# mapbox/robosat

Hardware: AMD Instinct MI355X
Metric: 512x512 tiles/sec train+predict, 1/2/4/8 MI355X; mIoU vs CPU ref (higher is better)
Workload: dtype f32; 1 GPU; rs predict ResNet50-UNet, bs=16 3x512x512 fp32 per GPU, 2 classes (BASELINE configs[1]); parallelism=tiles sharded over 1 rank(s), no collective

## Files before the change

### robosat_amd/csrc/common.h

```cpp
#pragma once
#include <hip/hip_runtime.h>
#include <stdint.h>

#include "../../include/robosat_hip.h"

typedef float f32x4 __attribute__((ext_vector_type(4)));
typedef float f32x16 __attribute__((ext_vector_type(16)));
typedef __bf16 bf16_t;
typedef __bf16 bf16x4 __attribute__((ext_vector_type(4)));
typedef __bf16 bf16x8 __attribute__((ext_vector_type(8)));
typedef unsigned int u32x2 __attribute__((ext_vector_type(2)));
typedef unsigned int u32x4 __attribute__((ext_vector_type(4)));
typedef short s16x4 __attribute__((ext_vector_type(4)));
typedef short s16x8 __attribute__((ext_vector_type(8)));

__device__ __forceinline__ f32x4 rs_ld4(const float* p) { return *reinterpret_cast<const f32x4*>(p); }
__device__ __forceinline__ f32x4 rs_ld4(const bf16_t* p) {
  return __builtin_convertvector(*reinterpret_cast<const bf16x4*>(p), f32x4);
}
__device__ __forceinline__ void rs_st4(float* p, f32x4 v) { *reinterpret_cast<f32x4*>(p) = v; }
__device__ __forceinline__ void rs_st4(bf16_t* p, f32x4 v) {
  *reinterpret_cast<bf16x4*>(p) = __builtin_convertvector(v, bf16x4);
}
__device__ __forceinline__ float rs_ld1(const float* p) { return *p; }
__device__ __forceinline__ float rs_ld1(const bf16_t* p) { return (float)*p; }

template <int V>
struct rs_vecf {
  float v[V];
};
template <int V, typename T>
__device__ __forceinline__ rs_vecf<V> rs_ldv(const T* p) {
  rs_vecf<V> r;
  if constexpr (V == 4) {
    const f32x4 t = rs_ld4(p);
#pragma unroll
    for (int e = 0; e < 4; ++e) r.v[e] = t[e];
  } else if constexpr (sizeof(T) == 2) {
    const bf16x8 t = *reinterpret_cast<const bf16x8*>(p);
#pragma unroll
    for (int e = 0; e < 8; ++e) r.v[e] = (float)t[e];
  } else {
    const f32x4 a = *reinterpret_cast<const f32x4*>(p), b = *(reinterpret_cast<const f32x4*>(p) + 1);
#pragma unroll
    for (int e = 0; e < 4; ++e) r.v[e] = a[e], r.v[4 + e] = b[e];
  }
  return r;
}
template <int V, typename T>
__device__ __forceinline__ void rs_stv(T* p, const rs_vecf<V>& r) {
  if constexpr (V == 4) {
    rs_st4(p, f32x4{r.v[0], r.v[1], r.v[2], r.v[3]});
  } else if constexpr (sizeof(T) == 2) {
    bf16x8 t;
#pragma unroll
    for (int e = 0; e < 8; ++e) t[e] = (bf16_t)r.v[e];
    *reinterpret_cast<bf16x8*>(p) = t;
  } else {
    *reinterpret_cast<f32x4*>(p) = f32x4{r.v[0], r.v[1], r.v[2], r.v[3]};
    *(reinterpret_cast<f32x4*>(p) + 1) = f32x4{r.v[4], r.v[5], r.v[6], r.v[7]};
  }
}

__device__ __forceinline__ void rs_ld_row32(const bf16_t* p, float (&v)[32]) {
  bf16x8 t[4];
#pragma unroll
  for (int j = 0; j < 4; ++j) t[j] = *reinterpret_cast<const bf16x8*>(p + j * 8);
#pragma unroll
  for (int j = 0; j < 4; ++j)
#pragma unroll
    for (int e = 0; e < 8; ++e) v[j * 8 + e] = (float)t[j][e];
}
__device__ __forceinline__ void rs_ld_row32(const float* p, float (&v)[32]) {
  f32x4 t[8];
#pragma unroll
  for (int j = 0; j < 8; ++j) t[j] = *reinterpret_cast<const f32x4*>(p + j * 4);
#pragma unroll
  for (int j = 0; j < 8; ++j)
#pragma unroll
    for (int e = 0; e < 4; ++e) v[j * 4 + e] = t[j][e];
}
__device__ __forceinline__ void rs_st_row32(bf16_t* p, const float (&v)[32]) {
#pragma unroll
  for (int j = 0; j < 4; ++j) {
    bf16x8 t;
#pragma unroll
    for (int e = 0; e < 8; ++e) t[e] = (bf16_t)v[j * 8 + e];
    *reinterpret_cast<bf16x8*>(p + j * 8) = t;
  }
}
__device__ __forceinline__ void rs_st_row32(float* p, const float (&v)[32]) {
#pragma unroll
  for (int j = 0; j < 8; ++j) {
    f32x4 t;
#pragma unroll
    for (int e = 0; e < 4; ++e) t[e] = v[j * 4 + e];
    *reinterpret_cast<f32x4*>(p + j * 4) = t;
  }
}

#define RS_LAUNCH_RESULT() ((int)hipGetLastError())

__device__ __forceinline__ void rs_lds_writes_done() { asm volatile("s_waitcnt lgkmcnt(0)" ::: "memory"); }

__device__ __forceinline__ int rs_xcd_remap(int b, int nwg) {
  const int xcd = b & 7, k = b >> 3;
  const int q = nwg >> 3, r = nwg & 7;
  const int base = (xcd < r) ? xcd * (q + 1) : r * (q + 1) + (xcd - r) * q;
  return base + k;
}

__device__ __forceinline__ float rs_xor16_sum(float v) {
  float a = v, b = v;
  asm("s_nop 1\n\tv_permlane16_swap_b32 %0, %1" : "+v"(a), "+v"(b));
  return a + b;
}
__device__ __forceinline__ float rs_xor32_sum(float v) {
  float a = v, b = v;
  asm("s_nop 1\n\tv_permlane32_swap_b32 %0, %1" : "+v"(a), "+v"(b));
  return a + b;
}

__device__ __forceinline__ float rs_row16_sum(float v) {
  v += __builtin_bit_cast(float, __builtin_amdgcn_update_dpp(0, __builtin_bit_cast(int, v), 0x128, 0xf, 0xf, false));
  v += __builtin_bit_cast(float, __builtin_amdgcn_update_dpp(0, __builtin_bit_cast(int, v), 0x124, 0xf, 0xf, false));
  v += __builtin_bit_cast(float, __builtin_amdgcn_update_dpp(0, __builtin_bit_cast(int, v), 0x122, 0xf, 0xf, false));
  v += __builtin_bit_cast(float, __builtin_amdgcn_update_dpp(0, __builtin_bit_cast(int, v), 0x121, 0xf, 0xf, false));
  return v;
}

__device__ __forceinline__ float rs_wave_sum(float v) {
#pragma unroll
  for (int o = 32; o > 0; o >>= 1) v += __shfl_xor(v, o, 64);
  return v;
}

__device__ __forceinline__ double rs_wave_sum(double v) {
#pragma unroll
  for (int o = 32; o > 0; o >>= 1) v += __shfl_xor(v, o, 64);
  return v;
}

static inline int rs_cdiv(long a, long b) { return (int)((a + b - 1) / b); }

inline int rs_cu_count() {
  static const int n = [] {
    int dev = 0, cus = 0;
    if (hipGetDevice(&dev) != hipSuccess || hipDeviceGetAttribute(&cus, hipDeviceAttributeMultiprocessorCount, dev) != hipSuccess || cus <= 0)
      cus = 256;
    return cus;
  }();
  return n;
}

struct rs_fastdiv {
  unsigned int mul;
  unsigned int shift;
  unsigned int div;
};

static inline rs_fastdiv rs_make_fastdiv(unsigned int d) {
  rs_fastdiv f;
  unsigned int s = 0;
  while ((1ull << s) < d) ++s;
  f.shift = s;
  f.mul = (unsigned int)((((1ull << s) - d) << 32) / d + 1);
  f.div = d;
  return f;
}

__host__ __device__ __forceinline__ unsigned int rs_div(unsigned int n, const rs_fastdiv f) {
#if defined(__HIP_DEVICE_COMPILE__)
  return (__umulhi(n, f.mul) + n) >> f.shift;
#else
  return (unsigned int)((((unsigned long long)n * f.mul) >> 32) + n) >> f.shift;
#endif
}

struct RsKnobs {
  int conv_tile = -1;
  int conv_rowb = 0;
  int conv_big = 1;
  int conv_min256 = 384;
  int conv_halo = 1;
  int conv_halo_min = 192;
  int conv_halo512 = -1;
  int conv_splitk = -1;
  int conv1x1_ew = -1;
  int conv1x1_np = 0;
  int conv1x1_ew_bf16 = 0;
  int halo_ko = 0;
  int wgrad_f32_phase = 1;
  int wgrad_f32_dma = -1;
  int wgrad_f32_blocks = 2048;
  int wgrad_f32_wino = 1;
  int wgrad_f32_wino_blocks = 1024;
  int wgrad_f32_wino33 = 1;
  int wgrad_f32_wino33_blocks = 256;
  int wgrad_blocks = 96;
  int wgrad_blocks_phase = 1536;
  int wgrad_phase4 = 1;
  int wgrad_blocks_phase4 = 256;
  int wgrad_ring = 3;
  int lovasz_xcd = 1;
  int wino_wide = 1;
  int wino_pixel = 1;
  int grow_fused = 0;
};
__attribute__((visibility("hidden"))) RsKnobs& rs_knobs();

__attribute__((visibility("hidden"))) int rs_wgrad_thin_plan(const rs_conv_desc* d, int* blocks, int* slices);
__attribute__((visibility("hidden"))) int rs_wgrad_thin_launch(const rs_conv_desc* d, const void* dy, const void* src,
                                                               float* partial, void* stream);

__attribute__((visibility("hidden"))) int rs_conv_thin_bf16_launch(int mode, const void* src, const void* wgt, const void* mask,
                                                                   void* out, int N, int Hs, int Ws, int relu, void* stream);

__attribute__((visibility("hidden"))) long rs_reduce_scratch_floats(long n, int splits);
__attribute__((visibility("hidden"))) int rs_reduce_splits(const float* ws, float* out, long n, int splits, float* scratch,
                                                           void* stream);

__attribute__((visibility("hidden"))) int rs_conv_dma_f32(const rs_conv_desc* d, const float* src1, const float* src2,
                                                          const float* weight, const float* scale, const float* shift,
                                                          const float* residual, const float* relu_mask, float* out,
                                                          void* stream);
__attribute__((visibility("hidden"))) int rs_conv_dma_tile(const rs_conv_desc* d);
```

### robosat_amd/csrc/conv_wino_f32.hip

```cpp
#define RS_CONV_INSTANTIATE
#include "conv_igemm_dma_kernel.h"

namespace {

struct WinoArgs {
  const float* src1;
  const float* src2;
  const float* u;
  float* out;
  int N, Hs, Ws, C1, C2, Cout;
  int TY, TX;
  int BBY, BBX;
  int nsub;
  int ncb;
  int relu;
  float* out2;
  const float* mask1;
  const float* mask2;
  int csplit;
};

template <int PB, bool PIX = false>
struct WinoGeom {
  static constexpr int HW = PIX ? 10 : 2 * PB + 1;
  static constexpr int PITCH = HW;
  static constexpr int HALF = PB + 1;
  static constexpr int SBROWS = (HW * PITCH + 7) / 8 * 8;
};

template <int PB>
__device__ __forceinline__ int wino_lane_tile(int l) {
  if constexpr (PB == 8) return ((l & 1) << 1) | (((l >> 1) & 1) << 2) | ((l >> 2) & 1) | (l & 8);
  return ((l & 1) << 1) | (((l >> 1) & 1) << 3) | ((l >> 2) & 1) | (((l >> 3) & 1) << 2);
}
__device__ __forceinline__ int wino_lane_pixel_y(int l) { return l & 3; }
__device__ __forceinline__ int wino_lane_pixel_x(int l) { return (l >> 2) & 3; }
typedef float f32x2 __attribute__((ext_vector_type(2)));
__device__ __forceinline__ f32x2 pk_sub(f32x2 a, f32x2 b) {
  f32x2 d;
  asm("v_pk_add_f32 %0, %1, %2 neg_lo:[0,1] neg_hi:[0,1]" : "=v"(d) : "v"(a), "v"(b));
  return d;
}
__device__ __forceinline__ int wino_lane_now() {
  int l;
  asm volatile("v_mbcnt_lo_u32_b32 %0, -1, 0\n\tv_mbcnt_hi_u32_b32 %0, -1, %0" : "=v"(l));
  return l;
}
__device__ __forceinline__ int wino_swz(int row) { return (row ^ (row >> 1)) & 3; }

template <int PB, int TG, int CG, int NM = 2, bool DG = false, bool PIX = false>
__global__ __launch_bounds__(512, 1) void conv_wino_f32_kernel(const WinoArgs p) {
  using G = WinoGeom<PB, PIX>;
  constexpr int NW = TG * CG;
  static_assert(NW == 8, "8 waves");
  static_assert(!PIX || (PB == 8 && !DG), "the pixel form: forward, 64-row sub-blocks");
  constexpr bool PAR = !DG && !PIX;
  constexpr int BMT = 16 * TG, BN = 16 * NM * CG;
  constexpr int SB = BMT / (PB * PB);
  static_assert(SB * PB * PB == BMT, "whole sub-blocks per block");
  constexpr int AROWS = SB * G::SBROWS;
  constexpr int IA = (AROWS + 15) / 16, IB = 9 * BN / 16;
  constexpr int AROWS_PAD = IA * 16;
  constexpr int JA = (IA + NW - 1) / NW, JB = (IB + NW - 1) / NW;
  constexpr int NI = JA + JB;
  constexpr int STAGE = (AROWS_PAD + 9 * BN) * 64;
  constexpr int KC = 16;

  constexpr int NTR = (AROWS_PAD + 64 * NW - 1) / (64 * NW);
  __shared__ __attribute__((aligned(16))) unsigned char smem[2 * STAGE + 2 * AROWS_PAD * 4 + NTR * 64 * NW * 4];
  int* tabs = reinterpret_cast<int*>(smem + 2 * STAGE);

  int* trows = tabs + 2 * AROWS_PAD;
  const int tid = threadIdx.x, lane = tid & 63;
  const int wave = __builtin_amdgcn_readfirstlane(tid >> 6);
  const int tg = wave % TG, cg = wave / TG;
  const int per_img = p.BBY * p.BBX;
  const int Cin = p.C1 + p.C2;
  const int nk = Cin / KC;
  const int ntiles = ((p.nsub + SB - 1) / SB) * p.ncb * (PAR ? 4 : 1);
  const int first = rs_xcd_remap(blockIdx.x, gridDim.x);
  const int nitems = (ntiles - first + (int)gridDim.x - 1) / (int)gridDim.x * (DG ? 4 : 1);
  const unsigned int lds0 = __builtin_amdgcn_readfirstlane(rs_lds_addr(smem));
  const long img1 = (long)p.Hs * p.Ws * p.C1 * (DG ? 4 : 1), img2 = (long)p.Hs * p.Ws * p.C2;

  constexpr int SBS = SB <= 2 ? SB : 1;
  struct Item {
    int py, px, nblk, nfirst, sub0;
    int n[SBS], y0[SBS], x0[SBS];
    bool live[SBS];
  };
  const int uni_first = __builtin_amdgcn_readfirstlane(first), uni_grid = __builtin_amdgcn_readfirstlane((int)gridDim.x);
  const int d_step = PAR ? uni_grid >> 2 : uni_grid, d_parstep = DG ? 1 : uni_grid & 3;
  int d_par = PAR ? uni_first & 3 : 0;
  int d_mblk = (PAR ? uni_first >> 2 : uni_first) / p.ncb, d_nblk = (PAR ? uni_first >> 2 : uni_first) - d_mblk * p.ncb;
  const int dq = d_step / p.ncb, dr = d_step - dq * p.ncb;
  auto decode_next = [&](Item& s) __attribute__((always_inline)) {
    s.py = PIX ? 0 : d_par >> 1;
    s.px = PIX ? 0 : d_par & 1;
    if (!DG || d_par == 0) {
      s.nblk = d_nblk;
      const int sub0 = s.sub0 = d_mblk * SB;
      int n = __builtin_amdgcn_readfirstlane(sub0 / per_img);
      const int r2 = sub0 - n * per_img;
      int bby = __builtin_amdgcn_readfirstlane(r2 / p.BBX);
      int bbx = r2 - bby * p.BBX;
      s.nfirst = n;
#pragma unroll
      for (int sb = 0; sb < SBS; ++sb) {
        s.live[sb] = sub0 + sb < p.nsub;
        s.n[sb] = n;
        s.y0[sb] = (PIX ? 8 : 2 * PB) * bby - 1;
        s.x0[sb] = (PIX ? 8 : 2 * PB) * bbx - 1;
        if (++bbx == p.BBX) {
          bbx = 0;
          if (++bby == p.BBY) {
            bby = 0;
            ++n;
          }
        }
      }
    }
    int carry = 0;
    if constexpr (!PIX) {
      d_par += d_parstep;
      carry = d_par >> 2;
      d_par &= 3;
    }
    if (!DG || carry) {
      d_mblk += dq;
      d_nblk += dr + (PAR ? carry : 0);
      if (d_nblk >= p.ncb) {
        d_nblk -= p.ncb;
        ++d_mblk;
      }
    }
  };
  Item cur, nxt;
  decode_next(cur);
  nxt = cur;
  auto sub_block = [&](const Item& s, int sb, int& n, int& y0, int& x0, bool& live) __attribute__((always_inline)) {
    if constexpr (SB <= 2) {
      const bool one = SB > 1 && sb > 0;
      n = one ? s.n[SBS - 1] : s.n[0];
      y0 = one ? s.y0[SBS - 1] : s.y0[0];
      x0 = one ? s.x0[SBS - 1] : s.x0[0];
      live = one ? s.live[SBS - 1] : s.live[0];
    } else {
      const int sub = s.sub0 + sb;
      n = sub / per_img;
      const int r2 = sub - n * per_img, bby = r2 / p.BBX, bbx = r2 - bby * p.BBX;
      y0 = 2 * bby * PB - 1;
      x0 = 2 * bbx * PB - 1;
      live = sub < p.nsub;
    }
  };

#pragma unroll
  for (int e = 0; e < NTR; ++e) {
    const int rho = tid + 64 * NW * e;
    const int sb = rho / G::SBROWS, rem = rho - sb * G::SBROWS;
    const int hy = rem / G::PITCH, xs = rem - hy * G::PITCH;
    const int hx = PIX ? xs : xs < G::HALF ? 2 * xs : 2 * (xs - G::HALF) + 1;
    trows[rho] = ((rho < AROWS && hy < G::HW) ? hy << 16 : -(1 << 28)) | (hx << 8) | sb;
  }
  auto build_table = [&](const Item& s, int seq) __attribute__((always_inline)) {
    int* tab = tabs + (seq & 1) * AROWS_PAD;
    const int tnow = 64 * wave + wino_lane_now();
#pragma unroll
    for (int e = 0; e < NTR; ++e) {
      const int rho = tnow + 64 * NW * e;
      if (rho < AROWS_PAD) {
        int n, y0, x0;
        bool live;
        const int row = trows[rho];
        sub_block(s, row & 255, n, y0, x0, live);
        const int y = y0 + (PIX ? 0 : s.py) + (row >> 16), x = x0 + (PIX ? 0 : s.px) + ((row >> 8) & 255);
        const bool in = live && (unsigned)y < (unsigned)p.Hs && (unsigned)x < (unsigned)p.Ws;
        const int v = DG ? ((n - s.nfirst) * 2 * p.Hs + 2 * y + 1 - s.py) * (2 * p.Ws) + 2 * x + 1 - s.px
                         : ((n - s.nfirst) * p.Hs + y) * p.Ws + x;
        tab[rho] = in ? v : -1;
      }
    }
    rs_lds_writes_done();
  };

  const int ra = lane >> 2, pp = lane & 3;
  static_assert(128 % BN == 0, "a wave's filter pieces: the same cout, whole positions apart");
  int doff[JA], doffu, upos[JB];
  {
    const int w = 16 * wave + ra, xi = PIX ? 0 : w / BN, co = w - (w / BN) * BN;
    doffu = ((xi * p.Cout + co) * Cin) * 4 + ((pp ^ wino_swz(w)) & 3) * 16;
  }
  const int ustep = (128 / BN) * p.Cout * Cin * 4;
#pragma unroll
  for (int j = 0; j < JB; ++j) {
    const int fi = wave + NW * j, xi = fi < IB ? 16 * fi / BN : 8, r = xi / 3, c = xi - 3 * r;
    upos[j] = PIX ? __builtin_amdgcn_readfirstlane(((2 * (r == 2) + (c == 2)) * 9 + xi) * p.Cout * Cin * 4) : 0;
  }
  int f_seq = 0, f_kc = 0, f_g = 0;
  int f_nb = 0, f_nfirst = 0;
  __amdgpu_buffer_rsrc_t rsrcs = rs_dma_rsrc<kDmaClamp>(p.src1, 0);
  __amdgpu_buffer_rsrc_t rsrcu = PIX ? rs_dma_rsrc<kDmaClamp>(p.u, (long)36 * p.Cout * Cin * 4) : rsrcs;
  auto fetch_item = [&](const Item& s) __attribute__((always_inline)) {
    f_nfirst = s.nfirst;
    f_nb = s.nblk * BN * Cin * 4;
    if constexpr (!PIX) rsrcu = rs_dma_rsrc<kDmaClamp>(p.u + (long)(2 * s.py + s.px) * 9 * p.Cout * Cin, (long)9 * p.Cout * Cin * 4);
  };
  auto set_source = [&](bool src_first) __attribute__((always_inline)) {
    const int cb = (src_first ? p.C1 : p.C2) * 4;
    rsrcs = rs_dma_rsrc<kDmaClamp>(src_first ? p.src1 + f_nfirst * img1 : p.src2 + f_nfirst * img2,
                                   (long)(p.N - f_nfirst) * (src_first ? img1 : img2) * 4);
    const int* tab = tabs + (f_seq & 1) * AROWS_PAD;
    int pix[JA];
#pragma unroll
    for (int j = 0; j < JA; ++j) {
      const int ii = wave + NW * j;
      pix[j] = tab[16 * (ii < IA ? ii : IA - 1) + ra];
    }
#pragma unroll
    for (int j = 0; j < JA; ++j) {
      const int ii = wave + NW * j;
      const int rho = 16 * (ii < IA ? ii : IA - 1) + ra;
      doff[j] = pix[j] < 0 ? kDmaOOB : pix[j] * cb + ((pp ^ wino_swz(rho)) & 3) * 16;
    }
  };
  auto fetch_chunk = [&](auto interleave, bool past) __attribute__((always_inline)) {
    const int c0 = f_kc * KC;
    const bool src_first = c0 < p.C1;
    if (!past) {
      if (f_kc == 0) fetch_item(nxt);
      if (c0 == 0 || c0 == p.C1) set_source(src_first);
    }
    const unsigned int fL = lds0 + (f_g & 1) * STAGE;
    const int fsa = __builtin_amdgcn_readfirstlane((src_first ? c0 : c0 - p.C1) * 4), fsu = __builtin_amdgcn_readfirstlane(c0 * 4 + f_nb);
    interleave([&](int j) __attribute__((always_inline)) {
      if (j < JA) {
        const int ii = wave + NW * j;
        if (j < JA - 1 || JA * NW == IA || ii < IA) rs_dma16(rsrcs, fL + ii * 1024, doff[j], fsa);
      } else {
        const int fi = wave + NW * (j - JA);
        if (j < NI - 1 || JB * NW == IB || fi < IB) rs_dma16(rsrcu, fL + (IA + fi) * 1024, doffu, fsu + (PIX ? upos[j - JA] : (j - JA) * ustep));
      }
    });
    ++f_g;
    if (!past && ++f_kc == nk) {
      f_kc = 0;
      ++f_seq;
    }
  };

  const int l15 = lane & 15, pc = lane >> 4;
  const int t = 16 * tg + wino_lane_tile<PB>(l15);
  const int tsb = 16 * tg / (PB * PB), tq = t - tsb * (PB * PB);
  const int tty = tq / PB, ttx = tq - tty * PB;
  const int wby = (tg >> 1) & 1, wbx = tg & 1;
  int addrA[3][3];
  {
    const int rho0 = PIX ? tsb * G::SBROWS + (4 * wby + wino_lane_pixel_y(l15)) * G::PITCH + 4 * wbx + wino_lane_pixel_x(l15)
                         : tsb * G::SBROWS + 2 * tty * G::PITCH + ttx;
#pragma unroll
    for (int r = 0; r < 3; ++r)
#pragma unroll
      for (int c = 0; c < 3; ++c) {
        const int rho = rho0 + r * G::PITCH + (PIX ? c : c == 0 ? 0 : (c == 1 ? G::HALF : 1));
        addrA[r][c] = rho * 64 + ((pc ^ wino_swz(rho)) & 3) * 16;
      }
  }
  const int addrB = AROWS_PAD * 64 + (16 * NM * cg + l15) * 64 + ((pc ^ wino_swz(l15)) & 3) * 16;

  build_table(cur, 0);
  __syncthreads();
  fetch_chunk([&](auto issue) __attribute__((always_inline)) {
#pragma unroll
    for (int j = 0; j < NI; ++j) issue(j);
  }, false);
  const int total = nitems * nk;
  const int Ho = 2 * p.Hs, Wo = 2 * p.Ws;

#if defined(RS_WINO_TAIL2) || defined(RS_WINO_TAIL4)
#ifndef RS_WINO_TAIL2
#define RS_WINO_TAIL2 (PIX ? 0 : PB == 4 ? 2 : (DG || TG == 8) ? 0 : 1)
#endif
#ifndef RS_WINO_TAIL4
#define RS_WINO_TAIL4 (PIX ? 0 : 1)
#endif
  constexpr int TAIL = NM >= 4 ? RS_WINO_TAIL4 : RS_WINO_TAIL2;
#else
  constexpr int TAIL = PIX ? 0 : NM >= 4 ? 1 : PB == 4 ? 2 : (DG || TG == 8) ? 0 : 1;
#endif
  static_assert(TAIL >= 0 && TAIL <= 2, "positions behind the barrier");
  constexpr int NMMA = 36 * NM, NHEAD = (9 - TAIL) * 4 * NM, NT = TAIL * 4 * NM;
  constexpr int PSTEP = 2 * NMMA / 3 / NI >= 1 ? 2 * NMMA / 3 / NI : 1;
  static_assert((NI - 1) * PSTEP < NHEAD, "the DMA pieces go out in the chunk's head");
  f32x4 V[9], Bq[9][NM];
  auto chunk_head = [&](const unsigned char* L, f32x4(&Vn)[9], f32x4(&B0)[NM], auto tail, auto nt) __attribute__((always_inline)) {
    constexpr int N = decltype(nt)::value, LEAD = N / 2;
    f32x4 P[3][3];
#pragma unroll
    for (int r = 0; r < 3; ++r)
#pragma unroll
      for (int c = 0; c < 3; ++c) P[r][c] = *reinterpret_cast<const f32x4*>(L + addrA[r][c]);
    __builtin_amdgcn_sched_barrier(0);
#pragma unroll
    for (int i = 0; i < LEAD; ++i) tail(i);
    __builtin_amdgcn_sched_barrier(0);
    f32x2 Tl[3][3], Th[3][3];
#pragma unroll
    for (int s = 0; s < 6; ++s) {
      if (s < 3) {
        const int r = s;
        const f32x2 l0 = {P[r][0][0], P[r][0][1]}, h0 = {P[r][0][2], P[r][0][3]};
        const f32x2 l1 = {P[r][1][0], P[r][1][1]}, h1 = {P[r][1][2], P[r][1][3]};
        const f32x2 l2 = {P[r][2][0], P[r][2][1]}, h2 = {P[r][2][2], P[r][2][3]};
        Tl[r][0] = pk_sub(l0, l1);
        Tl[r][1] = l1;
        Tl[r][2] = pk_sub(l2, l1);
        Th[r][0] = pk_sub(h0, h1);
        Th[r][1] = h1;
        Th[r][2] = pk_sub(h2, h1);
      } else {
        const int c = s - 3;
        const f32x2 a = pk_sub(Tl[0][c], Tl[1][c]), b = pk_sub(Tl[2][c], Tl[1][c]);
        const f32x2 d = pk_sub(Th[0][c], Th[1][c]), e = pk_sub(Th[2][c], Th[1][c]);
        Vn[0 * 3 + c] = f32x4{a[0], a[1], d[0], d[1]};
        Vn[1 * 3 + c] = f32x4{Tl[1][c][0], Tl[1][c][1], Th[1][c][0], Th[1][c][1]};
        Vn[2 * 3 + c] = f32x4{b[0], b[1], e[0], e[1]};
      }
#pragma unroll
      for (int i = LEAD + (N - LEAD) * s / 7; i < LEAD + (N - LEAD) * (s + 1) / 7; ++i) tail(i);
      __builtin_amdgcn_sched_barrier(0);
    }
#pragma unroll
    for (int m = 0; m < NM; ++m) B0[m] = *reinterpret_cast<const f32x4*>(L + addrB + (16 * m) * 64);
    __builtin_amdgcn_sched_barrier(0);
#pragma unroll
    for (int i = LEAD + (N - LEAD) * 6 / 7; i < N; ++i) tail(i);
    __builtin_amdgcn_sched_barrier(0);
  };
  int g = 0;
  f32x4 acc[9][NM];
  auto mfma = [&](int q) __attribute__((always_inline)) {
    const int x = q / (4 * NM), k = (q / NM) % 4, m = q % NM;
    acc[x][m] = __builtin_amdgcn_mfma_f32_16x16x4f32(Bq[x][m][k], V[x][k], acc[x][m], 0, 0, 0);
  };
  rs_dma_wait();
  __syncthreads();
  chunk_head(smem, V, Bq[0], [](int) {}, std::integral_constant<int, 0>());

  for (int seq = 0; seq < nitems; ++seq) {
    if (!DG || (seq & 3) == 0) {
#pragma unroll
      for (int x = 0; x < 9; ++x)
#pragma unroll
        for (int m = 0; m < NM; ++m) acc[x][m] = f32x4{0.f, 0.f, 0.f, 0.f};
    }

    for (int kc = 0; kc < nk; ++kc, ++g) {
      const unsigned char* L = smem + (g & 1) * STAGE;
      const bool more = g + 1 < total;
      fetch_chunk([&](auto issue) __attribute__((always_inline)) {
#pragma unroll
        for (int x = 0; x < 9 - TAIL; ++x) {
#pragma unroll
          for (int xr = x + 1; xr < (x + 1 == 9 - TAIL ? 9 : x + 2); ++xr)
#pragma unroll
            for (int m = 0; m < NM; ++m) Bq[xr][m] = *reinterpret_cast<const f32x4*>(L + addrB + (xr * BN + 16 * m) * 64);
          __builtin_amdgcn_sched_barrier(0);
#pragma unroll
          for (int i = 0; i < 4 * NM; ++i) {
            const int q = x * 4 * NM + i;
            if (q % PSTEP == 0 && q / PSTEP < NI) issue(q / PSTEP);
            mfma(q);
          }
        }
      }, !more);
      if (kc == 0 && seq + 1 < nitems) {
        decode_next(nxt);
        build_table(nxt, seq + 1);
      }
      rs_lds_writes_done();
      rs_dma_wait();
      __syncthreads();
      f32x4 Vn[9], B0[NM];
      chunk_head(smem + ((g + 1) & 1) * STAGE, Vn, B0, [&](int i) __attribute__((always_inline)) { mfma(NHEAD + i); },
                 std::integral_constant<int, NT>());
#pragma unroll
      for (int x = 0; x < 9; ++x) V[x] = Vn[x];
#pragma unroll
      for (int m = 0; m < NM; ++m) Bq[0][m] = B0[m];
    }

    int e_n, e_y0, e_x0;
    bool e_live;
    sub_block(cur, tsb, e_n, e_y0, e_x0, e_live);
    const int e_lane = wino_lane_now(), e_pc = e_lane >> 4;
    const int e_tq = 16 * tg + wino_lane_tile<PB>(e_lane & 15) - tsb * (PB * PB), e_ty = e_tq / PB, e_tx = e_tq - e_ty * PB;
    const int a0 = e_y0 + 1 + 2 * e_ty, b0 = e_x0 + 1 + 2 * e_tx;
    if constexpr (DG) {
      if ((seq & 3) == 3 && e_live) {
        const int co = cur.nblk * BN + 16 * NM * cg + 4 * e_pc;
        const bool second = p.out2 != nullptr && cur.nblk * BN >= p.csplit;
        float* ob = second ? p.out2 : p.out;
        const float* mb = second ? p.mask2 : p.mask1;
        const int ostride = p.out2 ? (second ? p.Cout - p.csplit : p.csplit) : p.Cout;
        const int ocol = second ? co - p.csplit : co;
#pragma unroll
        for (int u = 0; u < 2; ++u)
#pragma unroll
          for (int v = 0; v < 2; ++v) {
            const int a = a0 + u, b = b0 + v;
            if (a >= p.Hs || b >= p.Ws) continue;
            const long o = ((long)(e_n * p.Hs + a) * p.Ws + b) * ostride + ocol;
#pragma unroll
            for (int m = 0; m < NM; ++m) {
              f32x4 y = (acc[u * 3 + v][m] + acc[u * 3 + v + 1][m]) + (acc[(u + 1) * 3 + v][m] + acc[(u + 1) * 3 + v + 1][m]);
              if (mb) {
                const f32x4 z = *reinterpret_cast<const f32x4*>(mb + o + 16 * m);
#pragma unroll
                for (int e = 0; e < 4; ++e) y[e] = z[e] > 0.f ? y[e] : 0.f;
              }
              *reinterpret_cast<f32x4*>(ob + o + 16 * m) = y;
            }
          }
      }
    } else if constexpr (PIX) {
      const int a = e_y0 + 1 + 4 * wby + wino_lane_pixel_y(e_lane & 15), b = e_x0 + 1 + 4 * wbx + wino_lane_pixel_x(e_lane & 15);
      if (e_live && a < p.Hs && b < p.Ws) {
        float* obase = p.out + cur.nblk * BN + 16 * NM * cg + 4 * e_pc + ((long)(e_n * Ho + 2 * a) * Wo + 2 * b) * p.Cout;
#pragma unroll
        for (int u = 0; u < 2; ++u)
#pragma unroll
          for (int v = 0; v < 2; ++v) {
            float* o = obase + ((long)u * Wo + v) * p.Cout;
#pragma unroll
            for (int m = 0; m < NM; ++m) {
              f32x4 y = (acc[u * 3 + v][m] + acc[u * 3 + v + 1][m]) + (acc[(u + 1) * 3 + v][m] + acc[(u + 1) * 3 + v + 1][m]);
              if (p.relu) {
#pragma unroll
                for (int e = 0; e < 4; ++e) y[e] = fmaxf(y[e], 0.f);
              }
              *reinterpret_cast<f32x4*>(o + 16 * m) = y;
            }
          }
      }
    } else if (e_live) {
      float* obase = p.out + cur.nblk * BN + 16 * NM * cg + 4 * e_pc;
#pragma unroll
      for (int u = 0; u < 2; ++u)
#pragma unroll
        for (int v = 0; v < 2; ++v) {
          const int a = a0 + u, b = b0 + v;
          if (a >= p.Hs || b >= p.Ws) continue;
          float* o = obase + ((long)(e_n * Ho + 2 * a + cur.py) * Wo + 2 * b + cur.px) * p.Cout;
#pragma unroll
          for (int m = 0; m < NM; ++m) {
            f32x4 y = (acc[u * 3 + v][m] + acc[u * 3 + v + 1][m]) + (acc[(u + 1) * 3 + v][m] + acc[(u + 1) * 3 + v + 1][m]);
            if (p.relu) {
#pragma unroll
              for (int e = 0; e < 4; ++e) y[e] = fmaxf(y[e], 0.f);
            }
            *reinterpret_cast<f32x4*>(o + 16 * m) = y;
          }
        }
    }
    cur = nxt;
  }
  rs_dma_wait();
}

__global__ void pack_wino_phase_weight_kernel(const float* __restrict__ w, float* __restrict__ u, int Cout, int Cin, long total) {
  const long i = (long)blockIdx.x * blockDim.x + threadIdx.x;
  if (i >= total) return;
  const int ci = (int)(i % Cin);
  const long r = i / Cin;
  const int co = (int)(r % Cout), ph = (int)(r / Cout);
  const float* g = w + (((long)ph * Cout + co) * 4) * Cin + ci;
  const float g00 = g[0], g01 = g[Cin], g10 = g[2 * (long)Cin], g11 = g[3 * (long)Cin];
  const float v[9] = {g00, g00 + g01, g01, g00 + g10, (g00 + g01) + (g10 + g11), g01 + g11, g10, g10 + g11, g11};
#pragma unroll
  for (int x = 0; x < 9; ++x) u[(((long)ph * 9 + x) * Cout + co) * Cin + ci] = v[x];
}

__global__ void pack_wino_dgrad_weight_kernel(const float* __restrict__ wd, float* __restrict__ u, int Cin, int Cout, long total) {
  const long i = (long)blockIdx.x * blockDim.x + threadIdx.x;
  if (i >= total) return;
  const int co = (int)(i % Cout);
  const long r = i / Cout;
  const int ci = (int)(r % Cin), ph = (int)(r / Cin), py = ph >> 1, px = ph & 1;
  const float* g = wd + (long)ci * 16 * Cout + co;
  const float g00 = g[(long)(py * 4 + px) * Cout], g01 = g[(long)(py * 4 + 2 + px) * Cout];
  const float g10 = g[(long)((2 + py) * 4 + px) * Cout], g11 = g[(long)((2 + py) * 4 + 2 + px) * Cout];
  const float v[9] = {g00, g00 + g01, g01, g00 + g10, (g00 + g01) + (g10 + g11), g01 + g11, g10, g10 + g11, g11};
#pragma unroll
  for (int x = 0; x < 9; ++x) u[(((long)ph * 9 + x) * Cin + ci) * Cout + co] = v[x];
}

bool wino_wide() {
  return rs_knobs().wino_wide != 0;
}

constexpr bool kWinoPixel64 = true, kWinoPixel32 = true;
bool wino_pixel(int wgn) { return (wgn == 2 ? kWinoPixel64 : kWinoPixel32) && rs_knobs().wino_pixel != 0; }

bool wino_wide_rule(long regions, int ncb, int units) {
  return wino_wide() && (regions + 1) / 2 * ncb * units >= 2L * rs_cu_count();
}

struct WinoPlan {
  int pb, wgn;
  int sb;
  bool pix;
  bool worth;
  bool wide;
};

bool wino_plan(const rs_conv_desc* d, WinoPlan* pl, bool fwd = true, bool upsampled = false) {
  if (!d || d->N <= 0 || d->Hs <= 0 || d->Ws <= 0 || d->C1 <= 0 || (d->C1 % 16) || d->C2 < 0 || (d->C2 % 16) || d->Cout <= 0 ||
      (d->Cout % 32))
    return false;
  if (!(d->ups == 1 && d->kh == 3 && d->kw == 3 && d->stride == 1 && d->pad == 1 && d->Ho == 2 * d->Hs && d->Wo == 2 * d->Ws)) return false;
  const int ty = (d->Hs + 1) / 2, tx = (d->Ws + 1) / 2;
  if (ty < 4 || tx < 4) return false;
  pl->pb = (ty >= 8 && tx >= 8) ? 8 : 4;
  pl->wgn = (d->Cout % 64 == 0) ? 2 : 1;
  pl->sb = 16 * (8 / pl->wgn) / (pl->pb * pl->pb);
  if (d->C1 + d->C2 < 32) return false;
  const long cmax = d->C1 > d->C2 ? d->C1 : d->C2;
  if ((long)(pl->sb + 1) * d->Hs * d->Ws * cmax * 4 >= (1L << 31)) return false;
  if ((long)9 * d->Cout * (d->C1 + d->C2) * 4 >= (1L << 31)) return false;
  if ((long)d->N * d->Ho * d->Wo >= (1L << 31)) return false;
  pl->pix = fwd && upsampled && pl->pb == 8 && wino_pixel(pl->wgn) && (long)4 * 9 * d->Cout * (d->C1 + d->C2) * 4 < (1L << 31);
  pl->worth = pl->pb == 8;
  pl->wide = pl->pb == 8 && pl->wgn == 2 && wino_wide_rule((long)d->N * rs_cdiv(d->Hs, 16) * rs_cdiv(d->Ws, 16), d->Cout / 64, 4);
  if (pl->wide) pl->sb = 2;
  return true;
}

}

extern "C" int rs_conv2d_phase_wino_ok(const rs_conv_desc* d) {
  WinoPlan pl;
  if (!wino_plan(d, &pl)) return 0;
  return pl.worth ? 1 : 2;
}

extern "C" const char* rs_conv2d_phase_wino_name(const rs_conv_desc* d) {
  WinoPlan pl;
  if (!wino_plan(d, &pl)) return "";
  if (pl.pb == 8) return pl.wide ? "conv_wino_f32<phase,p8,128x64>" : (pl.wgn == 2 ? "conv_wino_f32<phase,p8,64x64>" : "conv_wino_f32<phase,p8,128x32>");
  return pl.wgn == 2 ? "conv_wino_f32<phase,p4,64x64>" : "conv_wino_f32<phase,p4,128x32>";
}

extern "C" int rs_pack_wino_phase_weight(const float* w_phase, float* u, int Cout, int Cin, rs_stream_t stream) {
  if (!w_phase || !u || Cout <= 0 || Cin <= 0) return RS_EINVAL;
  const long total = 4L * Cout * Cin;
  pack_wino_phase_weight_kernel<<<rs_cdiv(total, 256), 256, 0, (hipStream_t)stream>>>(w_phase, u, Cout, Cin, total);
  return RS_LAUNCH_RESULT();
}

namespace {
int wino_fwd_launch(const rs_conv_desc* d, const float* src1, const float* src2, const float* u, float* out, rs_stream_t stream,
                    bool upsampled) {
  WinoPlan pl;
  if (!wino_plan(d, &pl, true, upsampled) || !src1 || !u || !out || (d->C2 > 0 && !src2)) return RS_EINVAL;
  WinoArgs a;
  a.src1 = src1;
  a.src2 = src2;
  a.u = u;
  a.out = out;
  a.N = d->N;
  a.Hs = d->Hs;
  a.Ws = d->Ws;
  a.C1 = d->C1;
  a.C2 = d->C2;
  a.Cout = d->Cout;
  a.TY = (d->Hs + 1) / 2;
  a.TX = (d->Ws + 1) / 2;
  a.BBY = pl.pix ? rs_cdiv(d->Hs, 8) : rs_cdiv(a.TY, pl.pb);
  a.BBX = pl.pix ? rs_cdiv(d->Ws, 8) : rs_cdiv(a.TX, pl.pb);
  if ((long)d->N * a.BBY * a.BBX >= (1L << 31)) return RS_EINVAL;
  a.nsub = d->N * a.BBY * a.BBX;
  a.ncb = d->Cout / (32 * pl.wgn);
  a.relu = d->relu;
  a.out2 = nullptr;
  a.mask1 = a.mask2 = nullptr;
  a.csplit = 0;
  const long items = (long)rs_cdiv(a.nsub, pl.sb) * a.ncb * (pl.pix ? 1 : 4);
  if (items >= (1L << 31)) return RS_EINVAL;
  const int grid = (int)(items < rs_cu_count() ? items : rs_cu_count());
  hipStream_t s = (hipStream_t)stream;
  if (pl.pix && pl.wide) conv_wino_f32_kernel<8, 8, 1, 4, false, true><<<grid, 512, 0, s>>>(a);
  else if (pl.pix && pl.wgn == 2) conv_wino_f32_kernel<8, 4, 2, 2, false, true><<<grid, 512, 0, s>>>(a);
  else if (pl.pix) conv_wino_f32_kernel<8, 8, 1, 2, false, true><<<grid, 512, 0, s>>>(a);
  else if (pl.wide) conv_wino_f32_kernel<8, 8, 1, 4><<<grid, 512, 0, s>>>(a);
  else if (pl.pb == 8 && pl.wgn == 2) conv_wino_f32_kernel<8, 4, 2><<<grid, 512, 0, s>>>(a);
  else if (pl.pb == 8) conv_wino_f32_kernel<8, 8, 1><<<grid, 512, 0, s>>>(a);
  else if (pl.wgn == 2) conv_wino_f32_kernel<4, 4, 2><<<grid, 512, 0, s>>>(a);
  else conv_wino_f32_kernel<4, 8, 1><<<grid, 512, 0, s>>>(a);
  return RS_LAUNCH_RESULT();
}
}

extern "C" int rs_conv2d_fwd_phase_wino(const rs_conv_desc* d, const float* src1, const float* src2, const float* u, float* out,
                                        rs_stream_t stream) {
  return wino_fwd_launch(d, src1, src2, u, out, stream, false);
}

extern "C" int rs_conv2d_fwd_upsampled_wino(const rs_conv_desc* d, const float* src1, const float* src2, const float* u, float* out,
                                            rs_stream_t stream) {
  return wino_fwd_launch(d, src1, src2, u, out, stream, true);
}

namespace {
bool wino_dgrad_plan(const rs_conv_desc* d, rs_conv_desc* g, WinoPlan* pl) {
  if (!d || d->C1 <= 0 || d->C2 < 0 || d->Cout <= 0) return false;
  *g = *d;
  g->C1 = d->Cout;
  g->C2 = 0;
  g->Cout = d->C1 + d->C2;
  if (!wino_plan(g, pl, false) || !pl->worth) return false;
  if ((long)(pl->sb + 1) * 4 * d->Hs * d->Ws * g->C1 * 4 >= (1L << 31)) return false;
  if (g->Cout % 64) return false;
  pl->wide = wino_wide_rule((long)d->N * rs_cdiv(d->Hs, 16) * rs_cdiv(d->Ws, 16), g->Cout / 64, 1);
  pl->sb = pl->wide ? 2 : 1;
  return true;
}
}

extern "C" int rs_conv2d_dgrad_phase_wino_ok(const rs_conv_desc* d) {
  rs_conv_desc g;
  WinoPlan pl;
  return wino_dgrad_plan(d, &g, &pl) ? 1 : 0;
}

extern "C" const char* rs_conv2d_dgrad_phase_wino_name(const rs_conv_desc* d) {
  rs_conv_desc g;
  WinoPlan pl;
  if (!wino_dgrad_plan(d, &g, &pl)) return "";
  return pl.wide ? "conv_wino_f32<dgrad4x4,p8,128x64>" : "conv_wino_f32<dgrad4x4,p8,64x64>";
}

extern "C" int rs_pack_wino_dgrad_weight(const float* wd4x4, float* u, int Cin, int Cout, rs_stream_t stream) {
  if (!wd4x4 || !u || Cin <= 0 || Cout <= 0) return RS_EINVAL;
  const long total = 4L * Cin * Cout;
  pack_wino_dgrad_weight_kernel<<<rs_cdiv(total, 256), 256, 0, (hipStream_t)stream>>>(wd4x4, u, Cin, Cout, total);
  return RS_LAUNCH_RESULT();
}

extern "C" int rs_conv2d_dgrad_phase_wino(const rs_conv_desc* d, const float* dz, const float* u, float* out, const float* mask,
                                          float* out2, const float* mask2, int csplit, rs_stream_t stream) {
  rs_conv_desc g;
  WinoPlan pl;
  if (!wino_dgrad_plan(d, &g, &pl) || !dz || !u || !out) return RS_EINVAL;
  if (out2 ? (csplit <= 0 || csplit >= g.Cout || (csplit % 64) != 0) : (csplit != 0 || mask2 != nullptr)) return RS_EINVAL;
  WinoArgs a;
  a.src1 = dz;
  a.src2 = nullptr;
  a.u = u;
  a.out = out;
  a.out2 = out2;
  a.mask1 = mask;
  a.mask2 = mask2;
  a.csplit = csplit;
  a.N = d->N;
  a.Hs = d->Hs;
  a.Ws = d->Ws;
  a.C1 = g.C1;
  a.C2 = 0;
  a.Cout = g.Cout;
  a.TY = (d->Hs + 1) / 2;
  a.TX = (d->Ws + 1) / 2;
  a.BBY = rs_cdiv(a.TY, pl.pb);
  a.BBX = rs_cdiv(a.TX, pl.pb);
  a.nsub = d->N * a.BBY * a.BBX;
  a.ncb = g.Cout / 64;
  a.relu = 0;
  const bool wide = pl.wide;
  const long items = (long)rs_cdiv(a.nsub, pl.sb) * a.ncb;
  if (items >= (1L << 29)) return RS_EINVAL;
  const int grid = (int)(items < rs_cu_count() ? items : rs_cu_count());
  hipStream_t s = (hipStream_t)stream;
  if (wide) conv_wino_f32_kernel<8, 8, 1, 4, true><<<grid, 512, 0, s>>>(a);
  else conv_wino_f32_kernel<8, 4, 2, 2, true><<<grid, 512, 0, s>>>(a);
  return RS_LAUNCH_RESULT();
}
```

### robosat_amd/csrc/knobs.hip

```cpp
#include <stdio.h>
#include <stdlib.h>
#include <string.h>

#include "common.h"

namespace {

struct Entry {
  const char* name;
  const char* env;
  int RsKnobs::*field;
  int lo, hi;
};

bool in_range(const Entry& e, int v) {
  if (v < e.lo || v > e.hi) return false;
  if (e.field == &RsKnobs::conv_rowb) return v == 0 || v == 64 || v == 128;
  return true;
}

const Entry kEntries[] = {
    {"conv_tile", "RS_CONV_TILE", &RsKnobs::conv_tile, -1, 9},
    {"conv_rowb", "RS_CONV_ROWB", &RsKnobs::conv_rowb, 0, 128},
    {"conv_big", "RS_CONV_BIG", &RsKnobs::conv_big, 0, 1},
    {"conv_min256", "RS_CONV_MIN256", &RsKnobs::conv_min256, 0, 1048576},
    {"conv_halo", "RS_CONV_HALO", &RsKnobs::conv_halo, 0, 1},
    {"conv_halo_min", "RS_CONV_HALO_MIN", &RsKnobs::conv_halo_min, 0, 1048576},
    {"conv_halo512", "RS_CONV_HALO512", &RsKnobs::conv_halo512, -1, 1},
    {"conv_splitk", "RS_CONV_SPLITK", &RsKnobs::conv_splitk, -1, 16},
    {"conv1x1_ew", "RS_CONV1X1_EW", &RsKnobs::conv1x1_ew, -1, 1},
    {"conv1x1_np", "RS_CONV1X1_NP", &RsKnobs::conv1x1_np, -1, 1},
    {"conv1x1_ew_bf16", "RS_CONV1X1_EW_BF16", &RsKnobs::conv1x1_ew_bf16, 0, 1},
    {"halo_ko", "RS_HALO_KO", &RsKnobs::halo_ko, 0, 4},
    {"wgrad_f32_phase", "RS_WGRAD_F32_PHASE", &RsKnobs::wgrad_f32_phase, 0, 1},
    {"wgrad_f32_dma", "RS_WGRAD_F32_DMA", &RsKnobs::wgrad_f32_dma, -1, 1},
    {"wgrad_f32_blocks", "RS_WGRAD_F32_BLOCKS", &RsKnobs::wgrad_f32_blocks, 1, 1048576},
    {"wgrad_f32_wino", "RS_WGRAD_F32_WINO", &RsKnobs::wgrad_f32_wino, 0, 1},
    {"wgrad_f32_wino_blocks", "RS_WGRAD_F32_WINO_BLOCKS", &RsKnobs::wgrad_f32_wino_blocks, 1, 1048576},
    {"wgrad_f32_wino33", "RS_WGRAD_F32_WINO33", &RsKnobs::wgrad_f32_wino33, 0, 1},
    {"wgrad_f32_wino33_blocks", "RS_WGRAD_F32_WINO33_BLOCKS", &RsKnobs::wgrad_f32_wino33_blocks, 1, 1048576},
    {"wgrad_blocks", "RS_WGRAD_BLOCKS", &RsKnobs::wgrad_blocks, 1, 1048576},
    {"wgrad_blocks_phase", "RS_WGRAD_BLOCKS_PHASE", &RsKnobs::wgrad_blocks_phase, 1, 1048576},
    {"wgrad_phase4", "RS_WGRAD_PHASE4", &RsKnobs::wgrad_phase4, 0, 1},
    {"wgrad_blocks_phase4", "RS_WGRAD_BLOCKS_PHASE4", &RsKnobs::wgrad_blocks_phase4, 1, 1048576},
    {"wgrad_ring", "RS_WGRAD_RING", &RsKnobs::wgrad_ring, 2, 7},
    {"lovasz_xcd", "RS_LOVASZ_XCD", &RsKnobs::lovasz_xcd, 0, 1},
    {"wino_wide", "ROBOSAT_WINO_WIDE", &RsKnobs::wino_wide, 0, 1},
    {"wino_pixel", "ROBOSAT_WINO_PIXEL", &RsKnobs::wino_pixel, 0, 1},
    {"grow_fused", "RS_GROW_FUSED", &RsKnobs::grow_fused, 0, 16},
};

}

RsKnobs& rs_knobs() {
  static RsKnobs k = [] {
    RsKnobs v;
    for (const Entry& e : kEntries)
      if (const char* s = getenv(e.env)) {
        const int x = atoi(s);
        if (in_range(e, x)) v.*(e.field) = x;
        else fprintf(stderr, "robosat_hip: %s=%s is outside [%d, %d]: ignored, the rule stays\n", e.env, s, e.lo, e.hi);
      }
    return v;
  }();
  return k;
}

extern "C" int rs_set_knob(const char* name, int value) {
  if (!name) return RS_EINVAL;
  for (const Entry& e : kEntries)
    if (strcmp(name, e.name) == 0) {
      if (!in_range(e, value)) return RS_EINVAL;
      rs_knobs().*(e.field) = value;
      return 0;
    }
  return RS_EINVAL;
}

extern "C" int rs_get_knob(const char* name, int* value) {
  if (!name || !value) return RS_EINVAL;
  for (const Entry& e : kEntries)
    if (strcmp(name, e.name) == 0) {
      *value = rs_knobs().*(e.field);
      return 0;
    }
  return RS_EINVAL;
}
```

Baseline: 1756 tiles/s.

## Process two K-chunks per barrier in pixel Winograd forward kernel with four-stage LDS ring

```diff
diff --git a/robosat_amd/csrc/common.h b/robosat_amd/csrc/common.h
--- a/robosat_amd/csrc/common.h
+++ b/robosat_amd/csrc/common.h
@@ -205,6 +205,7 @@
   int lovasz_xcd = 1;
   int wino_wide = 1;
   int wino_pixel = 1;
+  int wino_cpb = 2;
   int grow_fused = 0;
 };
 __attribute__((visibility("hidden"))) RsKnobs& rs_knobs();
diff --git a/robosat_amd/csrc/conv_wino_f32.hip b/robosat_amd/csrc/conv_wino_f32.hip
--- a/robosat_amd/csrc/conv_wino_f32.hip
+++ b/robosat_amd/csrc/conv_wino_f32.hip
@@ -48,12 +48,14 @@
 }
 __device__ __forceinline__ int wino_swz(int row) { return (row ^ (row >> 1)) & 3; }
 
-template <int PB, int TG, int CG, int NM = 2, bool DG = false, bool PIX = false>
+template <int PB, int TG, int CG, int NM = 2, bool DG = false, bool PIX = false, int CPB = 1>
 __global__ __launch_bounds__(512, 1) void conv_wino_f32_kernel(const WinoArgs p) {
   using G = WinoGeom<PB, PIX>;
   constexpr int NW = TG * CG;
   static_assert(NW == 8, "8 waves");
   static_assert(!PIX || (PB == 8 && !DG), "the pixel form: forward, 64-row sub-blocks");
+  static_assert(CPB == 1 || (CPB == 2 && PIX && NM == 2), "two chunks per barrier: the NM = 2 pixel forms");
+  constexpr int NST = 2 * CPB;
   constexpr bool PAR = !DG && !PIX;
   constexpr int BMT = 16 * TG, BN = 16 * NM * CG;
   constexpr int SB = BMT / (PB * PB);
@@ -67,8 +69,9 @@
   constexpr int KC = 16;
 
   constexpr int NTR = (AROWS_PAD + 64 * NW - 1) / (64 * NW);
-  __shared__ __attribute__((aligned(16))) unsigned char smem[2 * STAGE + 2 * AROWS_PAD * 4 + NTR * 64 * NW * 4];
-  int* tabs = reinterpret_cast<int*>(smem + 2 * STAGE);
+  static_assert(NST * STAGE + 2 * AROWS_PAD * 4 + NTR * 64 * NW * 4 <= 160 * 1024, "the block's LDS");
+  __shared__ __attribute__((aligned(16))) unsigned char smem[NST * STAGE + 2 * AROWS_PAD * 4 + NTR * 64 * NW * 4];
+  int* tabs = reinterpret_cast<int*>(smem + NST * STAGE);
 
   int* trows = tabs + 2 * AROWS_PAD;
   const int tid = threadIdx.x, lane = tid & 63;
@@ -231,7 +234,7 @@
       if (f_kc == 0) fetch_item(nxt);
       if (c0 == 0 || c0 == p.C1) set_source(src_first);
     }
-    const unsigned int fL = lds0 + (f_g & 1) * STAGE;
+    const unsigned int fL = lds0 + (f_g & (NST - 1)) * STAGE;
     const int fsa = __builtin_amdgcn_readfirstlane((src_first ? c0 : c0 - p.C1) * 4), fsu = __builtin_amdgcn_readfirstlane(c0 * 4 + f_nb);
     interleave([&](int j) __attribute__((always_inline)) {
       if (j < JA) {
@@ -274,6 +277,11 @@
 #pragma unroll
     for (int j = 0; j < NI; ++j) issue(j);
   }, false);
+  if constexpr (CPB == 2)
+    fetch_chunk([&](auto issue) __attribute__((always_inline)) {
+#pragma unroll
+      for (int j = 0; j < NI; ++j) issue(j);
+    }, false);
   const int total = nitems * nk;
   const int Ho = 2 * p.Hs, Wo = 2 * p.Ws;
 
@@ -355,7 +363,65 @@
         for (int m = 0; m < NM; ++m) acc[x][m] = f32x4{0.f, 0.f, 0.f, 0.f};
     }
 
-    for (int kc = 0; kc < nk; ++kc, ++g) {
+    for (int kc = 0; kc < nk; kc += CPB, g += CPB) {
+      if constexpr (CPB == 2) {
+#ifndef RS_WINO_CPB_TAIL
+#define RS_WINO_CPB_TAIL 1
+#endif
+        constexpr int CT = RS_WINO_CPB_TAIL;
+        static_assert(TAIL == 0 && CT >= 0 && CT <= 2, "positions around the inner head");
+        constexpr int QS = NI * PSTEP, QH = (9 - CT) * 4 * NM;
+        static_assert(QS <= QH && (2 * NI - 1) * PSTEP < 2 * NMMA, "the second chunk's pieces: from A's main positions on, inside the interval");
+        const unsigned char* LA = smem + (g & (NST - 1)) * STAGE;
+        const unsigned char* LB = LA + STAGE;
+        const bool more = g + CPB < total;
+        auto qstep = [&](int Q, bool reads, auto issue, int pbase) __attribute__((always_inline)) {
+          const int c = Q / NMMA, q = Q - c * NMMA, x = q / (4 * NM);
+          if (reads && q % (4 * NM) == 0) {
+            const unsigned char* L = c ? LB : LA;
+            const int nmain = c ? 9 : 9 - CT;
+#pragma unroll
+            for (int xr = x + 1; xr < (x + 1 == nmain ? 9 : x + 2); ++xr)
+#pragma unroll
+              for (int m = 0; m < NM; ++m) Bq[xr][m] = *reinterpret_cast<const f32x4*>(L + addrB + (xr * BN + 16 * m) * 64);
+            __builtin_amdgcn_sched_barrier(0);
+          }
+          const int pj = Q / PSTEP - pbase;
+          if (Q % PSTEP == 0 && pj >= 0 && pj < NI) issue(pj);
+          mfma(q);
+        };
+        fetch_chunk([&](auto issue) __attribute__((always_inline)) {
+#pragma unroll
+          for (int Q = 0; Q < QS; ++Q) qstep(Q, true, issue, 0);
+        }, !more);
+        fetch_chunk([&](auto issue) __attribute__((always_inline)) {
+#pragma unroll
+          for (int Q = QS; Q < QH; ++Q) qstep(Q, true, issue, NI);
+          f32x4 Vn[9], B0[NM];
+          chunk_head(LB, Vn, B0, [&](int i) __attribute__((always_inline)) { qstep(QH + i, false, issue, NI); },
+                     std::integral_constant<int, CT * 4 * NM>());
+#pragma unroll
+          for (int x = 0; x < 9; ++x) V[x] = Vn[x];
+#pragma unroll
+          for (int m = 0; m < NM; ++m) Bq[0][m] = B0[m];
+#pragma unroll
+          for (int Q = NMMA; Q < 2 * NMMA; ++Q) qstep(Q, true, issue, NI);
+        }, !more);
+        if (kc == 0 && seq + 1 < nitems) {
+          decode_next(nxt);
+          build_table(nxt, seq + 1);
+        }
+        rs_lds_writes_done();
+        rs_dma_wait();
+        __syncthreads();
+        f32x4 Vn[9], B0[NM];
+        chunk_head(smem + ((g + CPB) & (NST - 1)) * STAGE, Vn, B0, [](int) {}, std::integral_constant<int, 0>());
+#pragma unroll
+        for (int x = 0; x < 9; ++x) V[x] = Vn[x];
+#pragma unroll
+        for (int m = 0; m < NM; ++m) Bq[0][m] = B0[m];
+        continue;
+      }
       const unsigned char* L = smem + (g & 1) * STAGE;
       const bool more = g + 1 < total;
       fetch_chunk([&](auto issue) __attribute__((always_inline)) {
@@ -512,6 +578,7 @@
   bool pix;
   bool worth;
   bool wide;
+  int cpb;
 };
 
 bool wino_plan(const rs_conv_desc* d, WinoPlan* pl, bool fwd = true, bool upsampled = false) {
@@ -533,6 +600,8 @@
   pl->worth = pl->pb == 8;
   pl->wide = pl->pb == 8 && pl->wgn == 2 && wino_wide_rule((long)d->N * rs_cdiv(d->Hs, 16) * rs_cdiv(d->Ws, 16), d->Cout / 64, 4);
   if (pl->wide) pl->sb = 2;
+  const int cin = d->C1 + d->C2;
+  pl->cpb = (pl->pix && pl->wgn == 1 && rs_knobs().wino_cpb != 1 && cin % 32 == 0 && cin >= 64) ? 2 : 1;
   return true;
 }
 
@@ -591,6 +660,7 @@
   hipStream_t s = (hipStream_t)stream;
   if (pl.pix && pl.wide) conv_wino_f32_kernel<8, 8, 1, 4, false, true><<<grid, 512, 0, s>>>(a);
   else if (pl.pix && pl.wgn == 2) conv_wino_f32_kernel<8, 4, 2, 2, false, true><<<grid, 512, 0, s>>>(a);
+  else if (pl.pix && pl.cpb == 2) conv_wino_f32_kernel<8, 8, 1, 2, false, true, 2><<<grid, 512, 0, s>>>(a);
   else if (pl.pix) conv_wino_f32_kernel<8, 8, 1, 2, false, true><<<grid, 512, 0, s>>>(a);
   else if (pl.wide) conv_wino_f32_kernel<8, 8, 1, 4><<<grid, 512, 0, s>>>(a);
   else if (pl.pb == 8 && pl.wgn == 2) conv_wino_f32_kernel<8, 4, 2><<<grid, 512, 0, s>>>(a);
diff --git a/robosat_amd/csrc/knobs.hip b/robosat_amd/csrc/knobs.hip
--- a/robosat_amd/csrc/knobs.hip
+++ b/robosat_amd/csrc/knobs.hip
@@ -47,6 +47,7 @@
     {"lovasz_xcd", "RS_LOVASZ_XCD", &RsKnobs::lovasz_xcd, 0, 1},
     {"wino_wide", "ROBOSAT_WINO_WIDE", &RsKnobs::wino_wide, 0, 1},
     {"wino_pixel", "ROBOSAT_WINO_PIXEL", &RsKnobs::wino_pixel, 0, 1},
+    {"wino_cpb", "ROBOSAT_WINO_CPB", &RsKnobs::wino_cpb, 1, 2},
     {"grow_fused", "RS_GROW_FUSED", &RsKnobs::grow_fused, 0, 16},
 };
 
```

New measurement: 1755 tiles/s (median of 3 runs). No clear change (-0.1%).
